# Komputerowe-Projektowanie-Lekow/pmarlo

Hardware: AMD Instinct MI355X
Metric: frames/sec featurize->TICA->k-means->T-matrix, 1Mx64 synth; ITS rel-err (higher is better)
Workload: dtype f64; 1 GPU; synthetic 1000000 frames x 64 f32 features per GPU (AR(1) latents), TICA->10, k=500 (10 Lloyd iterations), lag=10, row-normalised T; frames_per_gpu=1000000, features=64, tica_dim=10, k=500, lag=10, kmeans_iters=10, parallelism=shards1

## Files before the change

include/msmhip.h:

```cpp
#ifndef MSMHIP_H
#define MSMHIP_H

#include <stddef.h>
#include <stdint.h>

#ifdef __cplusplus
extern "C" {
#endif

typedef struct msm_ctx msm_ctx;
typedef struct msm_event msm_event;
typedef struct msm_graph msm_graph;

typedef enum {
    MSM_OK = 0,
    MSM_ERR_INVALID = 1,
    MSM_ERR_HIP = 2,
    MSM_ERR_NOMEM = 3,
    MSM_ERR_UNSUPPORTED = 4,
    MSM_ERR_NOCONV = 5
} msm_status;

typedef enum { MSM_F32 = 0, MSM_F64 = 1 } msm_dtype;

// ... 93 lines not shown
msm_status msm_lagged_moments_onesided(msm_ctx* ctx, const void* d_x, msm_dtype dtype, int64_t n, int F,
                                       int64_t ld, const int64_t* h_seg_start, const int64_t* h_seg_stop,
                                       int n_seg, int lag, const double* d_shift, int assume_finite,
                                       double* d_moments);

msm_status msm_onesided_tica_eigenvalues(msm_ctx* ctx, const double* d_moments, int F, double clip,
                                         double* d_eigvals);

msm_status msm_moments_from_lagged(msm_ctx* ctx, const void* d_x, msm_dtype dtype, int64_t n, int F, int64_t ld,
                                   const int64_t* h_seg_start, const int64_t* h_seg_stop, int n_seg, int lag,
                                   const double* d_shift, const double* d_moments, double* d_sums);

msm_status msm_tica_solve(msm_ctx* ctx, const double* d_moments, const double* d_scale, int F,
                          double epsilon, int kinetic_map, double* d_eigvals, double* d_coeffs,
                          double* d_mean, int* d_rank);

msm_status msm_project(msm_ctx* ctx, const void* d_x, msm_dtype dtype, int64_t n, int F, int64_t ld,
                       const double* d_mu, const double* d_inv_sigma, const double* d_mean2,
                       const double* d_w, int d, int64_t ldw, double* d_y, int64_t ldy, double* d_absmax);

msm_status msm_project_finite(msm_ctx* ctx, const void* d_x, msm_dtype dtype, int64_t n, int F, int64_t ld,
                              const double* d_mu, const double* d_inv_sigma, const double* d_mean2,
                              const double* d_w, int d, int64_t ldw, double* d_y, int64_t ldy, double* d_absmax);

msm_status msm_eigh(msm_ctx* ctx, const double* d_a, int n, double* d_w, double* d_v, int* d_sweeps);


msm_status msm_kmeans_assign(msm_ctx* ctx, const void* d_x, msm_dtype dtype, int64_t n, int d,
                             int64_t ld, const double* d_centers, int k,
                             const double* d_mean, const double* d_std,
// ... 150 lines not shown
```

pmarlo_amd/_lib.py:

```python

from __future__ import annotations

import ctypes as C
from pathlib import Path

__all__ = ["lib", "load", "LIB_PATH", "check", "MsmError", "DECLARED_SYMBOLS"]

LIB_PATH = Path(__file__).resolve().parent / "csrc" / "libmsmhip.so"

MSM_OK, MSM_ERR_INVALID, MSM_ERR_HIP, MSM_ERR_NOMEM, MSM_ERR_UNSUPPORTED, MSM_ERR_NOCONV = range(6)
MSM_F32, MSM_F64 = 0, 1


class MsmError(RuntimeError):
    """A HIP-side failure reported through the C ABI."""


_vp = C.c_void_p
_i32 = C.c_int
_i64 = C.c_int64
_sz = C.c_size_t
_f64 = C.c_double
_pp = C.POINTER(C.c_void_p)

# ... 26 lines not shown
    "msm_featurize_sasa": (_i32, [_vp, _vp, _i64, _i32, _vp, _vp, _i32, _vp]),
    "msm_hbond_presence": (_i32, [_vp, _vp, _i64, _i32, _vp, _i32, C.c_float, C.c_float, _vp]),
    "msm_dssp": (_i32, [_vp, _vp, _i64, _i32, _vp, _vp, _vp, _i32, _vp]),
    "msm_count_transitions": (_i32, [_vp, _vp, _i64, _vp, _vp, _i32, _i32, _i32, _i32, _vp, _vp]),
    "msm_count_transitions_weighted": (
        _i32, [_vp, _vp, _vp, _i64, _vp, _vp, _i32, _i32, _i32, _i32, _vp, _vp]),
    "msm_count_transitions_lagscan": (_i32, [_vp, _vp, _i64, _vp, _vp, _i32, _vp, _i32, _i32, _vp, _vp]),
    "msm_state_counts": (_i32, [_vp, _vp, _i64, _i32, _vp]),
    "msm_column_moments_partial": (_i32, [_vp, _vp, _i32, _i64, _i32, _i64, _vp, _vp, _vp]),
    "msm_moments_finalize": (_i32, [_vp, _vp, _vp, _i32, _i32, _vp, _vp, _vp]),
    "msm_column_moments": (_i32, [_vp, _vp, _i32, _i64, _i32, _i64, _i32, _vp, _vp, _vp]),
    "msm_column_minmax": (_i32, [_vp, _vp, _i32, _i64, _i32, _i64, _vp, _vp, _vp]),
    "msm_standardise_params": (_i32, [_vp, _vp, _vp, _i32, _f64, _i32, _vp, _vp, _vp]),
    "msm_lagged_moments": (_i32, [_vp, _vp, _i32, _i64, _i32, _i64, _vp, _vp, _i32, _i32, _vp, _i32, _vp]),
    "msm_tica_solve": (_i32, [_vp, _vp, _vp, _i32, _f64, _i32, _vp, _vp, _vp, _vp]),
    "msm_lagged_moments_reversible": (_i32, [_vp, _vp, _i32, _i64, _i32, _i64, _vp, _vp, _i32, _i32, _vp, _i32, _vp]),
    "msm_lagged_moments_onesided": (_i32, [_vp, _vp, _i32, _i64, _i32, _i64, _vp, _vp, _i32, _i32, _vp, _i32, _vp]),
    "msm_onesided_tica_eigenvalues": (_i32, [_vp, _vp, _i32, _f64, _vp]),
    "msm_moments_from_lagged": (_i32, [_vp, _vp, _i32, _i64, _i32, _i64, _vp, _vp, _i32, _i32, _vp, _vp, _vp]),
    "msm_project": (_i32, [_vp, _vp, _i32, _i64, _i32, _i64, _vp, _vp, _vp, _vp, _i32, _i64, _vp, _i64, _vp]),
    "msm_project_finite": (_i32, [_vp, _vp, _i32, _i64, _i32, _i64, _vp, _vp, _vp, _vp, _i32, _i64, _vp, _i64, _vp]),
    "msm_eigh": (_i32, [_vp, _vp, _i32, _vp, _vp, _vp]),
    "msm_kmeans_assign": (_i32, [_vp, _vp, _i32, _i64, _i32, _i64, _vp, _i32, _vp, _vp, _vp, _vp]),
    "msm_kmeans_fit": (_i32, [_vp, _vp, _i32, _i64, _i32, _i64, _vp, _vp, _i32, C.c_uint64, _i32, _i32, _f64, _vp, _vp]),
    "msm_kmeans_fit_begin": (
        _i32, [_vp, _vp, _i32, _i64, _i32, _i64, _vp, _vp, _i32, C.c_uint64, _i32, _f64, _f64, _vp, _vp, _i32]),
    "msm_kmeans_accumulate": (_i32, [_vp, _vp, _i32, _i64, _i32, _i64, _vp, _i32, _vp, _vp, _vp, _vp, _vp]),
    "msm_kmeans_update": (_i32, [_vp, _vp, _vp, _i32, _i32, _vp, _vp, _i32]),
    "msm_comm_unique_id": (_i32, [_vp, _sz]),
    "msm_comm_init": (_i32, [_vp, _i32, _i32, _vp, _sz, _pp]),
# ... 104 lines not shown
```

pmarlo_amd/csrc/eig.hip:

```cpp
#include "common.h"

#ifdef MSM_JACOBI_STAMPS
__device__ unsigned long long g_jacobi_stamps[8];
#define JSTAMP(i)                                                                          \
    do {                                                                                   \
        unsigned long long t__;                                                            \
        asm volatile("s_memtime %0\n\ts_waitcnt lgkmcnt(0)" : "=s"(t__)::"memory");       \
        acc__[i] += t__ - last__;                                                          \
        last__ = t__;                                                                      \
    } while (0)
#define JSTAMP_INIT unsigned long long acc__[8] = {0, 0, 0, 0, 0, 0, 0, 0}; unsigned long long last__; asm volatile("s_memtime %0\n\ts_waitcnt lgkmcnt(0)" : "=s"(last__)::"memory");
#define JSTAMP_FLUSH if (threadIdx.x == 0) { for (int i__ = 0; i__ < 8; ++i__) g_jacobi_stamps[i__] += acc__[i__]; }
#else
#define JSTAMP(i)
#define JSTAMP_INIT
#define JSTAMP_FLUSH
#endif

namespace {

constexpr int kEigThreads = 1024;
constexpr int kMaxPairs = 128;

struct JacobiShared {
// ... 528 lines not shown
    const int r1 = 8 * nblocks - 32;
    return __popc(w0 ^ (w0 >> 1)) + __popc(bits ^ ((bits >> 1) | ((w0 & 1u) << (r1 - 1))));
}

__device__ __forceinline__ double bcast_lane(double x, int j) {
    const long long b = __double_as_longlong(x);
    const int lo = __builtin_amdgcn_readlane((int)b, j), hi = __builtin_amdgcn_readlane((int)(b >> 32), j);
    return __longlong_as_double(((long long)hi << 32) | (unsigned)lo);
}
template <typename F>
__device__ __forceinline__ void hh_for_groups(int sub, int k, F&& body) {
#pragma unroll
    for (int g = 0; g < 2; ++g)
        if (sub + 32 * g + 24 > k) body(g);
}
__device__ __forceinline__ void householder_phase(double* A, double* QT, int n, TriShared* ts) {
    static_assert(kEigThreads == 1024, "householder_phase deals the rows of A and Q' over sixteen waves");
    constexpr int ld = kTriLd;
    const int lane = threadIdx.x & 63, wave = __builtin_amdgcn_readfirstlane(threadIdx.x >> 6);
    const bool in = lane < n;
    const bool is_a = wave < 8;
#ifdef MSM_TRI_NOQ
    const bool is_q = false;
#else
    const bool is_q = !is_a;
#endif
    const int sub = wave & 7;
    double* part = ts->part[wave];
    const double* parts = ts->part[is_a ? 0 : 8];
    double2* vw = ts->vw[sub];
    double m[8];
#pragma unroll
    for (int t = 0; t < 8; ++t) {
        const int j = sub + 8 * t;
        m[t] = (in && j < n) ? (is_a ? A[j * ld + lane] : (j == lane ? 1.0 : 0.0)) : 0.0;
    }
    auto q_partial = [&](int c) {
        if (__builtin_amdgcn_readfirstlane(ts->taupub[c & 1] != 0.0)) {
            const double* vp = ts->vpub[c & 1];
            double s0 = 0.0, s1 = 0.0;
// ... 31 lines not shown
        const double* rowc = A + c * ld;
        double xi = rowc[in ? lane : 0];
        const double alpha = rowc[c + 1];
        if (wave == 0 && lane == c) ts->d[c] = xi;
        const bool actc = in && lane > c;
        if (!actc) xi = 0.0;
        const double sigma = wave_sum_all(lane > c + 1 ? xi * xi : 0.0);
        const bool nz = sigma != 0.0;
        const double h2 = fma(alpha, alpha, sigma);
        const double rs = nr_rsqrt(nz ? h2 : 1.0);
        const double beta = nz ? -copysign(h2 * rs, alpha) : alpha;
        tau = nz ? (beta - alpha) * -copysign(rs, alpha) : 0.0;
        const double scal = nr_rcp(nz ? alpha - beta : 1.0);
        vi = actc ? (lane == c + 1 ? 1.0 : (nz ? xi * scal : 0.0)) : 0.0;
        if (wave == 0) {
            ts->vpub[c & 1][lane] = vi;
            if (lane == 0) { ts->e[c] = beta; ts->taupub[c & 1] = tau; }
        }
        vw[lane].x = vi;
    };
    LSTAMP_INIT
    double vi = 0.0, tau = 0.0;
    if (is_a && n > 2) reflector(0, vi, tau);
    for (int k = 0; k + 2 < n; ++k) {
        LSTAMP(16);
        const bool act = in && lane > k;
        if (is_a) {
            double s0 = 0.0, s1 = 0.0;
            hh_for_groups(sub, k, [&](int g) {
                double v[4];
#pragma unroll
                for (int u = 0; u < 4; ++u) v[u] = vw[sub + 32 * g + 8 * u].x;
// ... 119 lines not shown
        for (int t = 0; t < 8; ++t)
            if (lane == sub + 8 * t && lane < n) ts->inv[lane] = nr_rsqrt(m[t]);
    }
    __syncthreads();
    if (what == 1 && in) {
#pragma unroll
        for (int t = 0; t < 8; ++t) {
            const int i = sub + 8 * t;
            if (i < n) W[lane * ld + i] = m[t] * ts->inv[i];
        }
    }
    __syncthreads();
    return true;
}

__device__ __forceinline__ bool tridiag_eigh(double* A, double* Q, double* X, int n, int ld, TriShared* ts, double orth_tol) {
    const int tid = threadIdx.x, nt = blockDim.x, lane = tid & 63, wave = tid >> 6;
    if (n == 1) {
        if (tid == 0) { ts->lam[0] = A[0]; A[0] = 1.0; }
        __syncthreads();
        return true;
    }
    if (ld != kTriLd) return false;
    TSTAMP_INIT
    if (tid == 0) ts->bad = 0;
    __syncthreads();
    TSTAMP(0);
    householder_phase(A, Q, n, ts);
    TSTAMP(1);
    __syncthreads();
    TSTAMP(2);
    {
        const double dl = lane < n ? ts->d[lane] : 0.0, el = lane < n ? ts->e[lane] : 0.0;
        double an = fmax(fabs(dl), fabs(el));
#pragma unroll
        for (int off = 32; off > 0; off >>= 1) an = fmax(an, __shfl_xor(an, off, 64));
        double sc = 1.0;
        if (an > 0.0 && an < 1e300) { int ex; (void)frexp(an, &ex); sc = ldexp(1.0, -ex); }
        const double ds = dl * sc, es = el * sc;
        const double em = lane > 0 && lane < n ? ts->e[lane - 1] * sc : 0.0;
        const double rad = fabs(em) + (lane + 1 < n ? fabs(es) : 0.0);
        double gl = lane < n ? ds - rad : 1e300, gu = lane < n ? ds + rad : -1e300;
#pragma unroll
        for (int off = 32; off > 0; off >>= 1) {
            gl = fmin(gl, __shfl_xor(gl, off, 64));
            gu = fmax(gu, __shfl_xor(gu, off, 64));
        }
        __syncthreads();
        if (wave == 0) {
            if (lane < n) { ts->d[lane] = ds; ts->e[lane] = es; ts->de[lane] = make_double2(ds, em * em); }
            else ts->de[lane] = make_double2(8.0, 0.0);
            if (lane < 8) ts->de[kTriMax + lane] = make_double2(8.0, 0.0);
            if (lane == 0) {
                if (!(an < 1e300)) ts->bad = 1;
                ts->scale = sc;
                const double bn = fmax(fabs(gl), fabs(gu));
                const double pad = 4.0 * n * 2.220446049250313e-16 * bn + 1e-290;
                ts->gl = gl - pad;
                ts->gu = gu + pad;
            }
        }
    }
    __syncthreads();
    TSTAMP(3);
    if (ts->bad) return false;
    if (tid < 8 * kTriMax && wave * 8 < n) {
        const int i = tid >> 3, t = tid & 7;
        const int nblocks = (n + 7) >> 3;
        double lo = ts->gl, hi = ts->gu;
        const double frac = (double)(t + 1) * (1.0 / 9.0);
        for (int it = 0; it < 20; ++it) {
            const double x = fma(hi - lo, frac, lo);
            const int c = sturm_count(ts, nblocks, x);
            double nlo = c <= i ? x : lo, nhi = c > i ? x : hi;
            nlo = hw_max_f64(nlo, mov_dpp64<0xB1>(nlo)); nhi = hw_min_f64(nhi, mov_dpp64<0xB1>(nhi));
            nlo = hw_max_f64(nlo, mov_dpp64<0x4E>(nlo)); nhi = hw_min_f64(nhi, mov_dpp64<0x4E>(nhi));
            nlo = hw_max_f64(nlo, mov_dpp64<0x141>(nlo)); nhi = hw_min_f64(nhi, mov_dpp64<0x141>(nhi));
            lo = nlo;
            hi = nhi;
        }
        if (i < n && t == 0) ts->lam[i] = 0.5 * (lo + hi);
    }
    __syncthreads();
    TSTAMP(4);
    const double tiny = 1e-290;
    double* Xc = X + (lane < n ? lane : 0);
    double* Ac = A + (lane < n ? lane : 0);
    const double lamb = ts->lam[lane < n ? lane : 0];
    if (wave == 0 && lane < n) {
        double q = ts->de[0].x - lamb;
        Xc[0] = q;
        for (int j0 = 1; j0 < n; j0 += 8) {
            double2 r[8];
#pragma unroll
            for (int u = 0; u < 8; ++u) r[u] = ts->de[j0 + u];
#pragma unroll
            for (int u = 0; u < 8; ++u) {
                if (j0 + u < n) {
                    if (fabs(q) < tiny) q = -tiny;
                    q = fma(-r[u].y, nr_rcp(q), r[u].x - lamb);
                    Xc[(j0 + u) * ld] = q;
                }
            }
        }
    } else if (wave == 1 && lane < n) {
        double r = ts->de[n - 1].x - lamb;
        if (fabs(r) < tiny) r = -tiny;
        double ir = nr_rcp(r);
        Ac[(n - 1) * ld] = ir;
        for (int j0 = n - 2; j0 >= 0; j0 -= 8) {
            double dj[8], e2[8];
#pragma unroll
            for (int u = 0; u < 8; ++u) {
                const int j = j0 - u >= 0 ? j0 - u : 0;
                dj[u] = ts->de[j].x;
                e2[u] = ts->de[j + 1].y;
            }
#pragma unroll
            for (int u = 0; u < 8; ++u) {
                if (j0 - u >= 0) {
                    r = fma(-e2[u], ir, dj[u] - lamb);
                    if (fabs(r) < tiny) r = -tiny;
                    ir = nr_rcp(r);
                    Ac[(j0 - u) * ld] = ir;
                }
            }
        }
    }
    __syncthreads();
    int kk = n - 1;
    if (wave < 2 && lane < n) {
        double gbest = fabs(Xc[(n - 1) * ld]);
        for (int j0 = n - 2; j0 >= 0; j0 -= 8) {
            double g[8];
#pragma unroll
            for (int u = 0; u < 8; ++u) {
                const int j = j0 - u >= 0 ? j0 - u : 0;
                g[u] = fabs(fma(-ts->de[j + 1].y, Ac[(j + 1) * ld], Xc[j * ld]));
            }
#pragma unroll
            for (int u = 0; u < 8; ++u)
                if (j0 - u >= 0 && g[u] <= gbest) { gbest = g[u]; kk = j0 - u; }
        }
    }
    __syncthreads();
    if (wave == 0 && lane < n) {
        double z = 1.0, nrm2 = 1.0;
        for (int j0 = n - 2; j0 >= 0; j0 -= 8) {
            double f[8];
#pragma unroll
            for (int u = 0; u < 8; ++u) {
                const int j = j0 - u >= 0 ? j0 - u : 0;
                double qq = Xc[j * ld];
                if (fabs(qq) < tiny) qq = -tiny;
                f[u] = -(ts->e[j] * nr_rcp(qq));
            }
#pragma unroll
            for (int u = 0; u < 8; ++u) {
                if (j0 - u >= 0 && j0 - u < kk) {
                    z = f[u] * z;
                    Xc[(j0 - u) * ld] = z;
                    nrm2 = fma(z, z, nrm2);
                }
            }
        }
        Xc[kk * ld] = 1.0;
        ts->praw[lane] = nrm2;
    } else if (wave == 1 && lane < n) {
        double z = 1.0, nrm2 = 0.0;
        for (int j0 = 0; j0 + 1 < n; j0 += 8) {
            double f[8];
#pragma unroll
            for (int u = 0; u < 8; ++u) {
                const int j = j0 + u + 1 < n ? j0 + u : 0;
                f[u] = -(ts->e[j] * Ac[(j + 1) * ld]);
            }
#pragma unroll
            for (int u = 0; u < 8; ++u) {
                if (j0 + u + 1 < n && j0 + u >= kk) {
                    z = f[u] * z;
                    Xc[(j0 + u + 1) * ld] = z;
                    nrm2 = fma(z, z, nrm2);
                }
            }
        }
        ts->uq[lane] = nrm2;
    }
    __syncthreads();
    if (tid < n) {
        const double nrm2 = ts->praw[tid] + ts->uq[tid];
        const bool ok = nrm2 > 0.0 && nrm2 < 1e300;
        ts->inv[tid] = nr_rsqrt(ok ? nrm2 : 1.0);
        if (!ok) ts->bad = 1;
    }
    __syncthreads();
    TSTAMP(5);
    {
        double worst = 0.0;
        bool bad = false;
        for (int e0 = tid; e0 < n * n; e0 += nt) {
            const int j = e0 / n, i = e0 - j * n;
            const double x0 = X[j * ld + i];
            const double xm = j > 0 ? ts->e[j - 1] * X[(j - 1) * ld + i] : 0.0;
            const double xp = j + 1 < n ? ts->e[j] * X[(j + 1) * ld + i] : 0.0;
            const double tx = fma(ts->d[j] - ts->lam[i], x0, xm + xp) * ts->inv[i];
            bad = bad || !(fabs(tx) <= 1e-10);
        }
        const int jj = lane & 15, g = lane >> 4;
        const int tiles = (n + 15) >> 4;
        for (int t = wave; t < tiles * tiles; t += nt >> 6) {
            const int a0 = (t / tiles) * 16, b0 = (t - (t / tiles) * tiles) * 16;
            if (b0 > a0) continue;
            const bool aok = a0 + jj < n, bok = b0 + jj < n;
            const int ai = aok ? a0 + jj : 0, bi = bok ? b0 + jj : 0;
            const double sa = ts->inv[ai], sb = ts->inv[bi];
            tri_v4f64 acc = {0.0, 0.0, 0.0, 0.0};
            for (int k0 = 0; k0 < n; k0 += 16) {
                double a[4], b[4];
#pragma unroll
                for (int u = 0; u < 4; ++u) {
                    const bool kok = k0 + 4 * u + g < n;
                    const int k = kok ? k0 + 4 * u + g : 0;
                    a[u] = X[k * ld + ai] * sa;
                    b[u] = X[k * ld + bi] * sb;
                    if (!(aok && kok)) a[u] = 0.0;
                    if (!(bok && kok)) b[u] = 0.0;
                }
#pragma unroll
                for (int u = 0; u < 4; ++u) acc = __builtin_amdgcn_mfma_f64_16x16x4f64(a[u], b[u], acc, 0, 0, 0);
            }
#pragma unroll
            for (int r = 0; r < 4; ++r) {
                const int row = a0 + g + 4 * r, col = b0 + jj;
                if (row < n && col < n) worst = fmax(worst, fabs(acc[r] - (row == col ? 1.0 : 0.0)));
            }
        }
        if (bad) worst = 1e300;
#pragma unroll
        for (int off = 32; off > 0; off >>= 1) worst = fmax(worst, __shfl_xor(worst, off, 64));
        if (lane == 0) ts->red[wave] = worst;
        __syncthreads();
        worst = 0.0;
        for (int w = 0; w < nt / 64; ++w) worst = fmax(worst, ts->red[w]);
        TSTAMP(6);
        if (ts->bad || !(worst <= orth_tol)) return false;
    }
    mfma_mm<true, false>(A, Q, X, n, n, n, ld, ts->inv);
    if (tid < n) ts->lam[tid] /= ts->scale;
    __syncthreads();
    TSTAMP(7);
    return true;
}

struct TicaWork {
    double *A, *V, *B1, *B2, *ev, *mean, *isc;
    int* order;
};

template <int lds_mats>
__global__ __launch_bounds__(kEigThreads) void tica_solve_kernel(
    const double* __restrict__ mom, const double* __restrict__ scale, int n, int ld, double epsilon, int kinetic_map,
    TicaWork wk, double* __restrict__ out_eig, double* __restrict__ out_W, double* __restrict__ out_mean,
    int* __restrict__ out_rank) {
    extern __shared__ __attribute__((aligned(16))) unsigned char smem_raw[];
    __shared__ JacobiShared sh;
    __shared__ TriShared ts;
    const int tid = threadIdx.x, nt = blockDim.x;
    double* lds = reinterpret_cast<double*>(smem_raw);
    const size_t mat = (size_t)n * ld;
    double *A, *V, *B1, *B2;
    if constexpr (lds_mats >= 2) { A = lds; V = lds + mat; } else { A = wk.A; V = wk.V; }
    if constexpr (lds_mats >= 4) { B1 = lds + 2 * mat; B2 = lds + 3 * mat; } else { B1 = wk.B1; B2 = wk.B2; }

    const double* M00 = mom;
    const double* M0t = mom + (size_t)n * n;
    const double* sx = M0t + (size_t)n * n;
    const double* sy = sx + n;
// ... 102 lines not shown
        __syncthreads();
    }
    mfma_mm<false, false>(A, B1, B2, n, rank, n, ld);
    mfma_mm<true, false>(V, B2, A, rank, rank, n, ld);
    for (int e = tid; e < rank * rank; e += nt) {
        const int i = e / rank, j = e - i * rank;
        A[i * ld + j] = 0.5 * (V[i * ld + j] + V[j * ld + i]);
    }
    __syncthreads();
    KSTAMP(10);
    const double* Vec = V;
    bool fast = false;
    if (kFused && rank <= kTriMax) {
        for (int e = tid; e < rank * rank; e += nt) wk.A[e] = A[(e / rank) * ld + (e % rank)];
        __syncthreads();
        fast = tridiag_eigh(A, V, B1, rank, ld, &ts, 1e-11);
        if (fast) {
            for (int i = tid; i < rank; i += nt) wk.ev[i] = ts.lam[i];
            Vec = A;
        } else {
            __syncthreads();
            for (int e = tid; e < rank * rank; e += nt) A[(e / rank) * ld + (e % rank)] = wk.A[e];
        }
        __syncthreads();
    }
    if (!fast) {
        jacobi_eigh(A, V, rank, ld, &sh, 40);
        for (int i = tid; i < rank; i += nt) wk.ev[i] = A[i * ld + i];
    }
    __syncthreads();
// ... 18 lines not shown
            const int lane = tid & 63, wave = tid >> 6;
            for (int j = wave; j < rank; j += nt >> 6) {
                double best = lane < n ? fabs(B1[lane * ld + j]) : -1.0;
                int bi = lane;
                double val = lane < n ? B1[lane * ld + j] : 0.0;
#pragma unroll
                for (int off = 1; off < 64; off <<= 1) {
                    const double ob = __shfl_xor(best, off, 64), ov = __shfl_xor(val, off, 64);
                    const int oi = __shfl_xor(bi, off, 64);
                    if (ob > best || (ob == best && oi < bi)) { best = ob; bi = oi; val = ov; }
                }
                if (lane == 0) sgn[j] = val < 0.0 ? -1.0 : 1.0;
            }
        }
        __syncthreads();
        for (int e = tid; e < n * n; e += nt) {
            const int i = e / n, j = e - i * n;
            double v = 0.0;
            if (j < rank) {
                const int c = ord[j];
                v = B1[i * ld + c] * sgn[c];
                if (kinetic_map) v *= evl[c];
            }
            out_W[e] = v;
        }
        for (int j = tid; j < n; j += nt) out_eig[j] = j < rank ? evl[ord[j]] : 0.0;
        KSTAMP(12);
        return;
    }
    sort_desc_abs(wk.ev, rank, wk.order);
    mfma_mm<false, false>(B1, B2, Vec, n, rank, rank, ld);
    canonical_signs(B1, n, rank, ld);
    for (int e = tid; e < n * n; e += nt) {
        const int i = e / n, j = e - i * n;
        double v = 0.0;
        if (j < rank) {
            v = B1[i * ld + wk.order[j]];
            if (kinetic_map) v *= wk.ev[wk.order[j]];
        }
        out_W[e] = v;
    }
    for (int j = tid; j < n; j += nt) out_eig[j] = j < rank ? wk.ev[wk.order[j]] : 0.0;
    KSTAMP(12);
}

template <bool use_lds>
__global__ __launch_bounds__(kEigThreads) void eigh_kernel(const double* __restrict__ Ain, int n, int ld,
                                                          double* gA, double* gV, int* order,
                                                          double* __restrict__ out_w, double* __restrict__ out_v,
                                                          int* __restrict__ out_sweeps) {
    extern __shared__ __attribute__((aligned(16))) unsigned char smem_raw[];
    __shared__ JacobiShared sh;
    const int tid = threadIdx.x, nt = blockDim.x;
    double *A, *V;
    if constexpr (use_lds) { A = reinterpret_cast<double*>(smem_raw); V = A + (size_t)n * ld; }
    else { A = gA; V = gV; }
    for (int e = tid; e < n * n; e += nt) {
// ... 113 lines not shown
            const double b = gw[j];
            rank += (b > a) || (b == a && j < i);
        }
        order[rank] = i;
    }
    __syncthreads();
    for (int j = tid; j < n; j += nt) out_eig[j] = gw[order[j]];
}

size_t jacobi_lds_bytes(int n, int ld) { return (size_t)(n <= kTriMax ? 3 : 2) * n * ld * sizeof(double); }

}

extern "C" {

msm_status msm_tica_solve(msm_ctx* ctx, const double* d_moments, const double* d_scale, int F, double epsilon,
                          int kinetic_map, double* d_eigvals, double* d_coeffs, double* d_mean, int* d_rank) {
    if (!ctx) return MSM_ERR_INVALID;
    MSM_REQUIRE(ctx, F >= 1 && F <= 2 * kMaxPairs, "msm_tica_solve: need 1 <= F <= %d (got %d)", 2 * kMaxPairs, F);
    MSM_REQUIRE(ctx, epsilon >= 0.0, "msm_tica_solve: epsilon must be >= 0");
    MSM_REQUIRE(ctx, d_moments && d_eigvals && d_coeffs && d_mean && d_rank, "msm_tica_solve: NULL pointer");
    const int ld = F <= kTriMax ? kTriLd : (F | 1);
    const size_t mat = (size_t)F * ld;
    const size_t need = (4 * mat + 3 * F) * sizeof(double) + (size_t)F * sizeof(int) + 64;
    msm_status rs = msm_reserve_scratch(ctx, need);
    if (rs != MSM_OK) return rs;
    double* base = (double*)ctx->scratch;
    TicaWork wk;
    wk.A = base; wk.V = base + mat; wk.B1 = base + 2 * mat; wk.B2 = base + 3 * mat;
    wk.ev = base + 4 * mat; wk.mean = wk.ev + F; wk.isc = wk.mean + F; wk.order = (int*)(wk.isc + F);
    const size_t lds_budget = 150 * 1024;
    int lds_mats = 0;
    if (4 * mat * sizeof(double) <= lds_budget) lds_mats = 4;
    else if (2 * mat * sizeof(double) <= lds_budget) lds_mats = 2;
    const size_t lds = (size_t)lds_mats * mat * sizeof(double);
    auto kern = lds_mats == 4 ? tica_solve_kernel<4> : (lds_mats == 2 ? tica_solve_kernel<2> : tica_solve_kernel<0>);
    if (lds > 48 * 1024)
        MSM_HIP(ctx, hipFuncSetAttribute((const void*)kern, hipFuncAttributeMaxDynamicSharedMemorySize, (int)lds));
    hipLaunchKernelGGL(kern, dim3(1), dim3(kEigThreads), lds, ctx->stream, d_moments, d_scale, F, ld, epsilon,
                       kinetic_map, wk, d_eigvals, d_coeffs, d_mean, d_rank);
    MSM_CHECK_LAUNCH(ctx);
    return MSM_OK;
}

msm_status msm_onesided_tica_eigenvalues(msm_ctx* ctx, const double* d_moments, int F, double clip, double* d_eigvals) {
    if (!ctx) return MSM_ERR_INVALID;
    MSM_REQUIRE(ctx, F >= 1 && F <= 2 * kMaxPairs, "msm_onesided_tica_eigenvalues: need 1 <= F <= %d (got %d)",
                2 * kMaxPairs, F);
    MSM_REQUIRE(ctx, d_moments && d_eigvals && clip > 0.0, "msm_onesided_tica_eigenvalues: bad arguments");
    const int ld = F <= kTriMax ? kTriLd : (F | 1);
    const size_t mat = (size_t)F * ld;
    const size_t lds = 4 * mat * sizeof(double);
    const bool use_lds = lds <= 140 * 1024;
    msm_status rs = msm_reserve_scratch(ctx, ((use_lds ? 0 : 4 * mat) + (size_t)F * F + F) * sizeof(double) +
                                                 (size_t)F * sizeof(int) + 64);
    if (rs != MSM_OK) return rs;
    double* gP = (double*)ctx->scratch;
// ... 36 lines not shown
```

pmarlo_amd/device.py:

```python

from __future__ import annotations

import ctypes as C
import os
import sys
from typing import Iterable, Sequence

import numpy as np

from . import _lib
from ._lib import check, lib

__all__ = ["Engine", "DeviceArray", "get_engine", "segments_to_bounds"]


def _dtype_code(dtype: np.dtype) -> int:
    dtype = np.dtype(dtype)
    if dtype == np.float32:
        return _lib.MSM_F32
    if dtype == np.float64:
        return _lib.MSM_F64
    raise TypeError(f"feature matrices must be float32 or float64, got {dtype}")


# ... 425 lines not shown
        return out

    def moments_from_lagged(self, x: DeviceArray, lag: int, shift: DeviceArray, moments: DeviceArray, *, starts=None,
                            stops=None, out: DeviceArray | None = None) -> DeviceArray:
        n, F = x.shape
        if starts is None:
            starts, stops = segments_to_bounds(None, n)
        starts, stops = self._seg_ptrs(starts, stops)
        out = out if out is not None else self.empty((3 * F,), np.float64)
        check(lib.msm_moments_from_lagged(self.handle, x.ptr, _dtype_code(x.dtype), n, F, F, starts.ctypes.data,
                                          stops.ctypes.data, len(starts), int(lag), shift.ptr, moments.ptr, out.ptr),
              self.handle)
        return out

    def tica_solve(self, moments: DeviceArray, F: int, *, scale: DeviceArray | None = None,
                   epsilon: float = 1e-6, kinetic_map: bool = True, out=None):
        if out is not None:
            eig, W, mean, rank = out
        else:
            eig = self.empty((F,), np.float64)
            W = self.empty((F, F), np.float64)
            mean = self.empty((F,), np.float64)
            rank = self.empty((1,), np.int32)
        check(lib.msm_tica_solve(self.handle, moments.ptr, scale.ptr if scale is not None else None, F,
                                 float(epsilon), int(bool(kinetic_map)), eig.ptr, W.ptr, mean.ptr, rank.ptr),
              self.handle)
        return eig, W, mean, rank

    def project(self, x: DeviceArray, mu: DeviceArray, inv_sigma: DeviceArray, W: DeviceArray, d: int, *,
                mean2: DeviceArray | None = None, out: DeviceArray | None = None,
                absmax: DeviceArray | None = None, assume_finite: bool = False) -> DeviceArray:
        n, F = x.shape
        ldw = W.shape[1]
        out = out if out is not None else self.empty((n, d), np.float64)
        fn = lib.msm_project_finite if assume_finite else lib.msm_project
        check(fn(self.handle, x.ptr, _dtype_code(x.dtype), n, F, F, mu.ptr, inv_sigma.ptr,
                 mean2.ptr if mean2 is not None else None, W.ptr, int(d), ldw, out.ptr,
                 out.shape[1], absmax.ptr if absmax is not None else None), self.handle)
        return out

    def eigh(self, a: DeviceArray, want_vectors: bool = True):
# ... 548 lines not shown
```

pmarlo_amd/dist.py:

```python

from __future__ import annotations

import ctypes as C
import os
import time
from dataclasses import dataclass
from pathlib import Path

import numpy as np

from .device import DeviceArray, Engine

__all__ = ["Comm", "NativeComm", "TorchComm", "ShardedMSM", "ShardConfig", "exchange_shapes", "exchange_aliases",
           "torch_exchange_buffers", "bootstrap_id"]


class Comm:

    world = 1
    rank = 0

    def allreduce_sum(self, name: str) -> None: ...
    def allreduce_sum_from(self, name: str, src) -> None: ...
    def allreduce_min(self, name: str) -> None: ...
# ... 272 lines not shown
                raise ValueError("ShardConfig.pairs must list n_features atom pairs")
            self.xyz = x
            self.pairs_d = eng.to_device(np.ascontiguousarray(cfg.pairs, np.int32).reshape(F, 2))
            self.x = eng.empty((n, F), np.float32)
            eng.featurize_distances_into(self.xyz, self.pairs_d, self.x)
        else:
            self.xyz = None
            self.x = x
        if cfg.tica_dim > 0:
            self.mean, self.scale, self.inv_scale = (eng.empty((F,), np.float64) for _ in range(3))
            self.eig = eng.empty((F,), np.float64)
            self.W = eng.empty((F, F), np.float64)
            self.m2 = eng.empty((F,), np.float64)
            self.rank_d = eng.empty((1,), np.int32)
            self.Y = eng.empty((n, d), np.float64)
        else:
            self.Y = self.x
        self.labels = eng.empty((n,), np.int32)
        self.T = eng.empty((k, k), np.float64)
        self.rowsum = eng.empty((k,), np.float64)
        self.diag = eng.empty((1,), np.float64)
        self.km_sums = b["km_acc"].view((k * d,), np.int64)
        self.km_counts = b["km_acc"].view((k,), np.int64, offset_elems=k * d)
        multi_shard = self.comm is not None and (self.comm.world > 1 or self.always_exchange)
        self.km_local = eng.empty((k * d + k,), np.int64) if multi_shard else None
        nbytes = eng.kmeans_image_bytes(n, d)
        self.km_image = eng.empty((nbytes,), np.uint8) if nbytes else None
        self.accum_events: list = []
        self.stage_events: dict = {}
        self.time_accum = False
# ... 19 lines not shown
        multi = comm is not None and (comm.world > 1 or self.always_exchange)
        F, d, k = cfg.n_features, cfg.cluster_dim, cfg.k
        self._stamp("begin")
        if self.xyz is not None:
            eng.featurize_distances_into(self.xyz, self.pairs_d, self.x)
            self._stamp("featurize")
        if cfg.tica_dim > 0:
            eng.lagged_moments(self.x, cfg.lag, b["shift"], assume_finite=True, out=b["lagged"], symmetric=True)
            eng.moments_from_lagged(self.x, cfg.lag, b["shift"], b["lagged"], out=b["mom_sums"])
            if multi:
                comm.allreduce_sum("moments")
            eng.standardise_params(b["mom_sums"], b["shift"], F, float(self.n_total), True,
                                   out=(self.mean, self.scale, self.inv_scale))
            self._stamp("moments")
            eng.tica_solve(b["lagged"], F, scale=self.scale, epsilon=1e-6, kinetic_map=True,
                           out=(self.eig, self.W, self.m2, self.rank_d))
            self._stamp("tica_solve")
            eng.project(self.x, b["shift"], self.inv_scale, self.W, d, mean2=self.m2, out=self.Y,
                        absmax=b["fit_state"].view((1,), offset_elems=2), assume_finite=True)
            self._stamp("project")
        eng.kmeans_fit_begin(self.Y, k, seed=cfg.seed, n_total=self.n_total, tol2=0.0, centers=b["centers"],
                             state=b["fit_state"], absmax_ready=cfg.tica_dim > 0)
        if multi:
            if comm.rank != 0:
                b["centers"].fill_bytes_(0x7F)
            b["start_scale"].copy_from(b["fit_scale"])
            comm.allreduce_min("start")
            b["fit_scale"].copy_from(b["start_scale"])
            comm.reciprocal("fit_inv_scale", "fit_scale")
        acc = self.km_local if self.km_local is not None else b["km_acc"]
        acc.zero_()
# ... 57 lines not shown
```

Baseline: 653.7 million frames/s.

## Add leading-eigenpair TICA solve that computes only the kept components

```diff
diff --git a/include/msmhip.h b/include/msmhip.h
--- a/include/msmhip.h
+++ b/include/msmhip.h
@@ -131,6 +131,10 @@
 msm_status msm_tica_solve(msm_ctx* ctx, const double* d_moments, const double* d_scale, int F,
                           double epsilon, int kinetic_map, double* d_eigvals, double* d_coeffs,
                           double* d_mean, int* d_rank);
+
+msm_status msm_tica_solve_leading(msm_ctx* ctx, const double* d_moments, const double* d_scale, int F,
+                                  double epsilon, int kinetic_map, int n_keep, double* d_eigvals,
+                                  double* d_coeffs, double* d_mean, int* d_rank);
 
 msm_status msm_project(msm_ctx* ctx, const void* d_x, msm_dtype dtype, int64_t n, int F, int64_t ld,
                        const double* d_mu, const double* d_inv_sigma, const double* d_mean2,
diff --git a/pmarlo_amd/_lib.py b/pmarlo_amd/_lib.py
--- a/pmarlo_amd/_lib.py
+++ b/pmarlo_amd/_lib.py
@@ -64,6 +64,7 @@
     "msm_standardise_params": (_i32, [_vp, _vp, _vp, _i32, _f64, _i32, _vp, _vp, _vp]),
     "msm_lagged_moments": (_i32, [_vp, _vp, _i32, _i64, _i32, _i64, _vp, _vp, _i32, _i32, _vp, _i32, _vp]),
     "msm_tica_solve": (_i32, [_vp, _vp, _vp, _i32, _f64, _i32, _vp, _vp, _vp, _vp]),
+    "msm_tica_solve_leading": (_i32, [_vp, _vp, _vp, _i32, _f64, _i32, _i32, _vp, _vp, _vp, _vp]),
     "msm_lagged_moments_reversible": (_i32, [_vp, _vp, _i32, _i64, _i32, _i64, _vp, _vp, _i32, _i32, _vp, _i32, _vp]),
     "msm_lagged_moments_onesided": (_i32, [_vp, _vp, _i32, _i64, _i32, _i64, _vp, _vp, _i32, _i32, _vp, _i32, _vp]),
     "msm_onesided_tica_eigenvalues": (_i32, [_vp, _vp, _i32, _f64, _vp]),
diff --git a/pmarlo_amd/csrc/eig.hip b/pmarlo_amd/csrc/eig.hip
--- a/pmarlo_amd/csrc/eig.hip
+++ b/pmarlo_amd/csrc/eig.hip
@@ -566,6 +566,7 @@
     for (int g = 0; g < 2; ++g)
         if (sub + 32 * g + 24 > k) body(g);
 }
+template <bool kKeepQ = true>
 __device__ __forceinline__ void householder_phase(double* A, double* QT, int n, TriShared* ts) {
     static_assert(kEigThreads == 1024, "householder_phase deals the rows of A and Q' over sixteen waves");
     constexpr int ld = kTriLd;
@@ -575,7 +576,7 @@
 #ifdef MSM_TRI_NOQ
     const bool is_q = false;
 #else
-    const bool is_q = !is_a;
+    const bool is_q = kKeepQ && !is_a;
 #endif
     const int sub = wave & 7;
     double* part = ts->part[wave];
@@ -637,8 +638,13 @@
         const double scal = nr_rcp(nz ? alpha - beta : 1.0);
         vi = actc ? (lane == c + 1 ? 1.0 : (nz ? xi * scal : 0.0)) : 0.0;
         if (wave == 0) {
-            ts->vpub[c & 1][lane] = vi;
-            if (lane == 0) { ts->e[c] = beta; ts->taupub[c & 1] = tau; }
+            if constexpr (kKeepQ) {
+                ts->vpub[c & 1][lane] = vi;
+                if (lane == 0) ts->taupub[c & 1] = tau;
+            } else if (in) {
+                QT[c * ld + lane] = lane == c ? tau : vi;
+            }
+            if (lane == 0) ts->e[c] = beta;
         }
         vw[lane].x = vi;
     };
@@ -788,80 +794,64 @@
     return true;
 }
 
-__device__ __forceinline__ bool tridiag_eigh(double* A, double* Q, double* X, int n, int ld, TriShared* ts, double orth_tol) {
-    const int tid = threadIdx.x, nt = blockDim.x, lane = tid & 63, wave = tid >> 6;
-    if (n == 1) {
-        if (tid == 0) { ts->lam[0] = A[0]; A[0] = 1.0; }
-        __syncthreads();
-        return true;
-    }
-    if (ld != kTriLd) return false;
-    TSTAMP_INIT
-    if (tid == 0) ts->bad = 0;
-    __syncthreads();
-    TSTAMP(0);
-    householder_phase(A, Q, n, ts);
-    TSTAMP(1);
-    __syncthreads();
-    TSTAMP(2);
-    {
-        const double dl = lane < n ? ts->d[lane] : 0.0, el = lane < n ? ts->e[lane] : 0.0;
-        double an = fmax(fabs(dl), fabs(el));
-#pragma unroll
-        for (int off = 32; off > 0; off >>= 1) an = fmax(an, __shfl_xor(an, off, 64));
-        double sc = 1.0;
-        if (an > 0.0 && an < 1e300) { int ex; (void)frexp(an, &ex); sc = ldexp(1.0, -ex); }
-        const double ds = dl * sc, es = el * sc;
-        const double em = lane > 0 && lane < n ? ts->e[lane - 1] * sc : 0.0;
-        const double rad = fabs(em) + (lane + 1 < n ? fabs(es) : 0.0);
-        double gl = lane < n ? ds - rad : 1e300, gu = lane < n ? ds + rad : -1e300;
-#pragma unroll
-        for (int off = 32; off > 0; off >>= 1) {
-            gl = fmin(gl, __shfl_xor(gl, off, 64));
-            gu = fmax(gu, __shfl_xor(gu, off, 64));
-        }
-        __syncthreads();
-        if (wave == 0) {
-            if (lane < n) { ts->d[lane] = ds; ts->e[lane] = es; ts->de[lane] = make_double2(ds, em * em); }
-            else ts->de[lane] = make_double2(8.0, 0.0);
-            if (lane < 8) ts->de[kTriMax + lane] = make_double2(8.0, 0.0);
-            if (lane == 0) {
-                if (!(an < 1e300)) ts->bad = 1;
-                ts->scale = sc;
-                const double bn = fmax(fabs(gl), fabs(gu));
-                const double pad = 4.0 * n * 2.220446049250313e-16 * bn + 1e-290;
-                ts->gl = gl - pad;
-                ts->gu = gu + pad;
-            }
-        }
-    }
-    __syncthreads();
-    TSTAMP(3);
-    if (ts->bad) return false;
-    if (tid < 8 * kTriMax && wave * 8 < n) {
-        const int i = tid >> 3, t = tid & 7;
-        const int nblocks = (n + 7) >> 3;
-        double lo = ts->gl, hi = ts->gu;
-        const double frac = (double)(t + 1) * (1.0 / 9.0);
-        for (int it = 0; it < 20; ++it) {
-            const double x = fma(hi - lo, frac, lo);
-            const int c = sturm_count(ts, nblocks, x);
-            double nlo = c <= i ? x : lo, nhi = c > i ? x : hi;
-            nlo = hw_max_f64(nlo, mov_dpp64<0xB1>(nlo)); nhi = hw_min_f64(nhi, mov_dpp64<0xB1>(nhi));
-            nlo = hw_max_f64(nlo, mov_dpp64<0x4E>(nlo)); nhi = hw_min_f64(nhi, mov_dpp64<0x4E>(nhi));
-            nlo = hw_max_f64(nlo, mov_dpp64<0x141>(nlo)); nhi = hw_min_f64(nhi, mov_dpp64<0x141>(nhi));
-            lo = nlo;
-            hi = nhi;
-        }
-        if (i < n && t == 0) ts->lam[i] = 0.5 * (lo + hi);
-    }
-    __syncthreads();
-    TSTAMP(4);
+__device__ __forceinline__ void tri_scale_bounds(int n, TriShared* ts) {
+    const int lane = threadIdx.x & 63, wave = threadIdx.x >> 6;
+    const double dl = lane < n ? ts->d[lane] : 0.0, el = lane < n ? ts->e[lane] : 0.0;
+    double an = fmax(fabs(dl), fabs(el));
+#pragma unroll
+    for (int off = 32; off > 0; off >>= 1) an = fmax(an, __shfl_xor(an, off, 64));
+    double sc = 1.0;
+    if (an > 0.0 && an < 1e300) { int ex; (void)frexp(an, &ex); sc = ldexp(1.0, -ex); }
+    const double ds = dl * sc, es = el * sc;
+    const double em = lane > 0 && lane < n ? ts->e[lane - 1] * sc : 0.0;
+    const double rad = fabs(em) + (lane + 1 < n ? fabs(es) : 0.0);
+    double gl = lane < n ? ds - rad : 1e300, gu = lane < n ? ds + rad : -1e300;
+#pragma unroll
+    for (int off = 32; off > 0; off >>= 1) {
+        gl = fmin(gl, __shfl_xor(gl, off, 64));
+        gu = fmax(gu, __shfl_xor(gu, off, 64));
+    }
+    __syncthreads();
+    if (wave == 0) {
+        if (lane < n) { ts->d[lane] = ds; ts->e[lane] = es; ts->de[lane] = make_double2(ds, em * em); }
+        else ts->de[lane] = make_double2(8.0, 0.0);
+        if (lane < 8) ts->de[kTriMax + lane] = make_double2(8.0, 0.0);
+        if (lane == 0) {
+            if (!(an < 1e300)) ts->bad = 1;
+            ts->scale = sc;
+            const double bn = fmax(fabs(gl), fabs(gu));
+            const double pad = 4.0 * n * 2.220446049250313e-16 * bn + 1e-290;
+            ts->gl = gl - pad;
+            ts->gu = gu + pad;
+        }
+    }
+}
+
+__device__ __forceinline__ double multisect9(const TriShared* ts, int n, int i, int t) {
+    const int nblocks = (n + 7) >> 3;
+    double lo = ts->gl, hi = ts->gu;
+    const double frac = (double)(t + 1) * (1.0 / 9.0);
+    for (int it = 0; it < 20; ++it) {
+        const double x = fma(hi - lo, frac, lo);
+        const int c = sturm_count(ts, nblocks, x);
+        double nlo = c <= i ? x : lo, nhi = c > i ? x : hi;
+        nlo = hw_max_f64(nlo, mov_dpp64<0xB1>(nlo)); nhi = hw_min_f64(nhi, mov_dpp64<0xB1>(nhi));
+        nlo = hw_max_f64(nlo, mov_dpp64<0x4E>(nlo)); nhi = hw_min_f64(nhi, mov_dpp64<0x4E>(nhi));
+        nlo = hw_max_f64(nlo, mov_dpp64<0x141>(nlo)); nhi = hw_min_f64(nhi, mov_dpp64<0x141>(nhi));
+        lo = nlo;
+        hi = nhi;
+    }
+    return 0.5 * (lo + hi);
+}
+
+__device__ __forceinline__ void twisted_vectors(double* A, double* X, int n, int ncols, TriShared* ts) {
+    constexpr int ld = kTriLd;
+    const int tid = threadIdx.x, lane = tid & 63, wave = tid >> 6;
     const double tiny = 1e-290;
-    double* Xc = X + (lane < n ? lane : 0);
-    double* Ac = A + (lane < n ? lane : 0);
-    const double lamb = ts->lam[lane < n ? lane : 0];
-    if (wave == 0 && lane < n) {
+    double* Xc = X + (lane < ncols ? lane : 0);
+    double* Ac = A + (lane < ncols ? lane : 0);
+    const double lamb = ts->lam[lane < ncols ? lane : 0];
+    if (wave == 0 && lane < ncols) {
         double q = ts->de[0].x - lamb;
         Xc[0] = q;
         for (int j0 = 1; j0 < n; j0 += 8) {
@@ -877,7 +867,7 @@
                 }
             }
         }
-    } else if (wave == 1 && lane < n) {
+    } else if (wave == 1 && lane < ncols) {
         double r = ts->de[n - 1].x - lamb;
         if (fabs(r) < tiny) r = -tiny;
         double ir = nr_rcp(r);
@@ -903,7 +893,7 @@
     }
     __syncthreads();
     int kk = n - 1;
-    if (wave < 2 && lane < n) {
+    if (wave < 2 && lane < ncols) {
         double gbest = fabs(Xc[(n - 1) * ld]);
         for (int j0 = n - 2; j0 >= 0; j0 -= 8) {
             double g[8];
@@ -918,7 +908,7 @@
         }
     }
     __syncthreads();
-    if (wave == 0 && lane < n) {
+    if (wave == 0 && lane < ncols) {
         double z = 1.0, nrm2 = 1.0;
         for (int j0 = n - 2; j0 >= 0; j0 -= 8) {
             double f[8];
@@ -940,7 +930,7 @@
         }
         Xc[kk * ld] = 1.0;
         ts->praw[lane] = nrm2;
-    } else if (wave == 1 && lane < n) {
+    } else if (wave == 1 && lane < ncols) {
         double z = 1.0, nrm2 = 0.0;
         for (int j0 = 0; j0 + 1 < n; j0 += 8) {
             double f[8];
@@ -961,66 +951,192 @@
         ts->uq[lane] = nrm2;
     }
     __syncthreads();
-    if (tid < n) {
+    if (tid < ncols) {
         const double nrm2 = ts->praw[tid] + ts->uq[tid];
         const bool ok = nrm2 > 0.0 && nrm2 < 1e300;
         ts->inv[tid] = nr_rsqrt(ok ? nrm2 : 1.0);
         if (!ok) ts->bad = 1;
     }
     __syncthreads();
+}
+
+__device__ __forceinline__ double vectors_defect(const double* X, int n, int ncols, TriShared* ts) {
+    constexpr int ld = kTriLd;
+    const int tid = threadIdx.x, nt = blockDim.x, lane = tid & 63, wave = tid >> 6;
+    double worst = 0.0;
+    bool bad = false;
+    for (int e0 = tid; e0 < n * ncols; e0 += nt) {
+        const int j = e0 / ncols, i = e0 - j * ncols;
+        const double x0 = X[j * ld + i];
+        const double xm = j > 0 ? ts->e[j - 1] * X[(j - 1) * ld + i] : 0.0;
+        const double xp = j + 1 < n ? ts->e[j] * X[(j + 1) * ld + i] : 0.0;
+        const double tx = fma(ts->d[j] - ts->lam[i], x0, xm + xp) * ts->inv[i];
+        bad = bad || !(fabs(tx) <= 1e-10);
+    }
+    const int jj = lane & 15, g = lane >> 4;
+    const int tiles = (ncols + 15) >> 4;
+    for (int t = wave; t < tiles * tiles; t += nt >> 6) {
+        const int a0 = (t / tiles) * 16, b0 = (t - (t / tiles) * tiles) * 16;
+        if (b0 > a0) continue;
+        const bool aok = a0 + jj < ncols, bok = b0 + jj < ncols;
+        const int ai = aok ? a0 + jj : 0, bi = bok ? b0 + jj : 0;
+        const double sa = ts->inv[ai], sb = ts->inv[bi];
+        tri_v4f64 acc = {0.0, 0.0, 0.0, 0.0};
+        for (int k0 = 0; k0 < n; k0 += 16) {
+            double a[4], b[4];
+#pragma unroll
+            for (int u = 0; u < 4; ++u) {
+                const bool kok = k0 + 4 * u + g < n;
+                const int k = kok ? k0 + 4 * u + g : 0;
+                a[u] = X[k * ld + ai] * sa;
+                b[u] = X[k * ld + bi] * sb;
+                if (!(aok && kok)) a[u] = 0.0;
+                if (!(bok && kok)) b[u] = 0.0;
+            }
+#pragma unroll
+            for (int u = 0; u < 4; ++u) acc = __builtin_amdgcn_mfma_f64_16x16x4f64(a[u], b[u], acc, 0, 0, 0);
+        }
+#pragma unroll
+        for (int r = 0; r < 4; ++r) {
+            const int row = a0 + g + 4 * r, col = b0 + jj;
+            if (row < ncols && col < ncols) worst = fmax(worst, fabs(acc[r] - (row == col ? 1.0 : 0.0)));
+        }
+    }
+    if (bad) worst = 1e300;
+#pragma unroll
+    for (int off = 32; off > 0; off >>= 1) worst = fmax(worst, __shfl_xor(worst, off, 64));
+    if (lane == 0) ts->red[wave] = worst;
+    __syncthreads();
+    worst = 0.0;
+    for (int w = 0; w < nt / 64; ++w) worst = fmax(worst, ts->red[w]);
+    return worst;
+}
+
+__device__ __forceinline__ bool tridiag_eigh(double* A, double* Q, double* X, int n, int ld, TriShared* ts, double orth_tol) {
+    const int tid = threadIdx.x, wave = tid >> 6;
+    if (n == 1) {
+        if (tid == 0) { ts->lam[0] = A[0]; A[0] = 1.0; }
+        __syncthreads();
+        return true;
+    }
+    if (ld != kTriLd) return false;
+    TSTAMP_INIT
+    if (tid == 0) ts->bad = 0;
+    __syncthreads();
+    TSTAMP(0);
+    householder_phase(A, Q, n, ts);
+    TSTAMP(1);
+    __syncthreads();
+    TSTAMP(2);
+    tri_scale_bounds(n, ts);
+    __syncthreads();
+    TSTAMP(3);
+    if (ts->bad) return false;
+    if (tid < 8 * kTriMax && wave * 8 < n) {
+        const int i = tid >> 3, t = tid & 7;
+        const double lam = multisect9(ts, n, i, t);
+        if (i < n && t == 0) ts->lam[i] = lam;
+    }
+    __syncthreads();
+    TSTAMP(4);
+    twisted_vectors(A, X, n, n, ts);
     TSTAMP(5);
     {
-        double worst = 0.0;
-        bool bad = false;
-        for (int e0 = tid; e0 < n * n; e0 += nt) {
-            const int j = e0 / n, i = e0 - j * n;
-            const double x0 = X[j * ld + i];
-            const double xm = j > 0 ? ts->e[j - 1] * X[(j - 1) * ld + i] : 0.0;
-            const double xp = j + 1 < n ? ts->e[j] * X[(j + 1) * ld + i] : 0.0;
-            const double tx = fma(ts->d[j] - ts->lam[i], x0, xm + xp) * ts->inv[i];
-            bad = bad || !(fabs(tx) <= 1e-10);
-        }
-        const int jj = lane & 15, g = lane >> 4;
-        const int tiles = (n + 15) >> 4;
-        for (int t = wave; t < tiles * tiles; t += nt >> 6) {
-            const int a0 = (t / tiles) * 16, b0 = (t - (t / tiles) * tiles) * 16;
-            if (b0 > a0) continue;
-            const bool aok = a0 + jj < n, bok = b0 + jj < n;
-            const int ai = aok ? a0 + jj : 0, bi = bok ? b0 + jj : 0;
-            const double sa = ts->inv[ai], sb = ts->inv[bi];
-            tri_v4f64 acc = {0.0, 0.0, 0.0, 0.0};
-            for (int k0 = 0; k0 < n; k0 += 16) {
-                double a[4], b[4];
-#pragma unroll
-                for (int u = 0; u < 4; ++u) {
-                    const bool kok = k0 + 4 * u + g < n;
-                    const int k = kok ? k0 + 4 * u + g : 0;
-                    a[u] = X[k * ld + ai] * sa;
-                    b[u] = X[k * ld + bi] * sb;
-                    if (!(aok && kok)) a[u] = 0.0;
-                    if (!(bok && kok)) b[u] = 0.0;
-                }
-#pragma unroll
-                for (int u = 0; u < 4; ++u) acc = __builtin_amdgcn_mfma_f64_16x16x4f64(a[u], b[u], acc, 0, 0, 0);
-            }
-#pragma unroll
-            for (int r = 0; r < 4; ++r) {
-                const int row = a0 + g + 4 * r, col = b0 + jj;
-                if (row < n && col < n) worst = fmax(worst, fabs(acc[r] - (row == col ? 1.0 : 0.0)));
-            }
-        }
-        if (bad) worst = 1e300;
-#pragma unroll
-        for (int off = 32; off > 0; off >>= 1) worst = fmax(worst, __shfl_xor(worst, off, 64));
-        if (lane == 0) ts->red[wave] = worst;
-        __syncthreads();
-        worst = 0.0;
-        for (int w = 0; w < nt / 64; ++w) worst = fmax(worst, ts->red[w]);
+        const double worst = vectors_defect(X, n, n, ts);
         TSTAMP(6);
         if (ts->bad || !(worst <= orth_tol)) return false;
     }
     mfma_mm<true, false>(A, Q, X, n, n, n, ld, ts->inv);
     if (tid < n) ts->lam[tid] /= ts->scale;
+    __syncthreads();
+    TSTAMP(7);
+    return true;
+}
+
+__device__ __forceinline__ bool tridiag_leading(double* A, double* R, double* X, int n, int nk, TriShared* ts, int* sel,
+                                                double orth_tol) {
+    constexpr int ld = kTriLd;
+    const int tid = threadIdx.x, lane = tid & 63, wave = tid >> 6;
+    TSTAMP_INIT
+    if (tid == 0) ts->bad = 0;
+    __syncthreads();
+    TSTAMP(0);
+    householder_phase<false>(A, R, n, ts);
+    TSTAMP(1);
+    __syncthreads();
+    TSTAMP(2);
+    tri_scale_bounds(n, ts);
+    __syncthreads();
+    TSTAMP(3);
+    if (ts->bad) return false;
+    const int nb = nk + 1;
+    const int ncand = 2 * nb >= n ? n : 2 * nb;
+    auto cand = [&](int c) { return (ncand == n || c < nb) ? c : n - 2 * nb + c; };
+    if (wave * 64 < 8 * ncand) {
+        const int c = tid >> 3, t = tid & 7;
+        const int i = c < ncand ? cand(c) : 0;
+        const double lam = multisect9(ts, n, i, t);
+        if (c < ncand && t == 0) ts->lam[i] = lam;
+    }
+    __syncthreads();
+    TSTAMP(4);
+    if (tid < ncand) {
+        const int i = cand(tid);
+        const double li = ts->lam[i], a = fabs(li);
+        int r = 0;
+        for (int c = 0; c < ncand; ++c) {
+            const int j = cand(c);
+            const double b = fabs(ts->lam[j]);
+            r += (b > a) || (b == a && j < i);
+        }
+        if (r < nk) {
+            sel[r] = i;
+            const double gap = 1e-6 * fmax(fabs(ts->gl), fabs(ts->gu));
+            bool ok = ncand == n || (i != nk && i != n - 1 - nk);
+            if (ok && i > 0) ok = fabs(li - ts->lam[i - 1]) > gap;
+            if (ok && i + 1 < n) ok = fabs(ts->lam[i + 1] - li) > gap;
+            if (!ok) ts->bad = 1;
+        }
+    }
+    __syncthreads();
+    if (ts->bad) return false;
+    {
+        const double ls = tid < nk ? ts->lam[sel[tid]] : 0.0;
+        __syncthreads();
+        if (tid < nk) ts->lam[tid] = ls;
+        __syncthreads();
+    }
+    twisted_vectors(A, X, n, nk, ts);
+    TSTAMP(5);
+    {
+        const double worst = vectors_defect(X, n, nk, ts);
+        TSTAMP(6);
+        if (ts->bad || !(worst <= orth_tol)) return false;
+    }
+    if (wave < nk) {
+        const int ncol = (nk - wave + 15) >> 4;
+        const int row = lane < n ? lane : 0;
+        double x[4];
+#pragma unroll
+        for (int u = 0; u < 4; ++u) {
+            const int c = u < ncol ? wave + 16 * u : wave;
+            x[u] = lane < n ? X[row * ld + c] * ts->inv[c] : 0.0;
+        }
+        for (int k = n - 3; k >= 0; --k) {
+            const double* vk = R + k * ld;
+            const double tau = vk[k];
+            const double v = (lane > k && lane < n) ? vk[row] : 0.0;
+#pragma unroll
+            for (int u = 0; u < 4; ++u)
+                if (u < ncol) x[u] = fma(-tau * wave_sum_all(v * x[u]), v, x[u]);
+        }
+        if (lane < n) {
+#pragma unroll
+            for (int u = 0; u < 4; ++u)
+                if (u < ncol) A[lane * ld + wave + 16 * u] = x[u];
+        }
+    }
+    if (tid < nk) ts->lam[tid] /= ts->scale;
     __syncthreads();
     TSTAMP(7);
     return true;
@@ -1034,7 +1150,7 @@
 template <int lds_mats>
 __global__ __launch_bounds__(kEigThreads) void tica_solve_kernel(
     const double* __restrict__ mom, const double* __restrict__ scale, int n, int ld, double epsilon, int kinetic_map,
-    TicaWork wk, double* __restrict__ out_eig, double* __restrict__ out_W, double* __restrict__ out_mean,
+    int n_keep, TicaWork wk, double* __restrict__ out_eig, double* __restrict__ out_W, double* __restrict__ out_mean,
     int* __restrict__ out_rank) {
     extern __shared__ __attribute__((aligned(16))) unsigned char smem_raw[];
     __shared__ JacobiShared sh;
@@ -1167,6 +1283,44 @@
     if (kFused && rank <= kTriMax) {
         for (int e = tid; e < rank * rank; e += nt) wk.A[e] = A[(e / rank) * ld + (e % rank)];
         __syncthreads();
+        if (full_rank && n_keep < rank) {
+            if (tridiag_leading(A, V, B1, rank, n_keep, &ts, sh.q, 1e-11)) {
+                KSTAMP(11);
+                mfma_mm<false, false>(B1, B2, A, n, n_keep, n, ld);
+                double* sgn = ts.uq;
+                {
+                    const int lane = tid & 63, wave = tid >> 6;
+                    for (int j = wave; j < n_keep; j += nt >> 6) {
+                        double best = lane < n ? fabs(B1[lane * ld + j]) : -1.0;
+                        int bi = lane;
+                        double val = lane < n ? B1[lane * ld + j] : 0.0;
+#pragma unroll
+                        for (int off = 1; off < 64; off <<= 1) {
+                            const double ob = __shfl_xor(best, off, 64), ov = __shfl_xor(val, off, 64);
+                            const int oi = __shfl_xor(bi, off, 64);
+                            if (ob > best || (ob == best && oi < bi)) { best = ob; bi = oi; val = ov; }
+                        }
+                        if (lane == 0) sgn[j] = val < 0.0 ? -1.0 : 1.0;
+                    }
+                }
+                __syncthreads();
+                for (int e = tid; e < n * n; e += nt) {
+                    const int i = e / n, j = e - i * n;
+                    double v = 0.0;
+                    if (j < n_keep) {
+                        v = B1[i * ld + j] * sgn[j];
+                        if (kinetic_map) v *= ts.lam[j];
+                    }
+                    out_W[e] = v;
+                }
+                for (int j = tid; j < n; j += nt) out_eig[j] = j < n_keep ? ts.lam[j] : 0.0;
+                KSTAMP(12);
+                return;
+            }
+            __syncthreads();
+            for (int e = tid; e < rank * rank; e += nt) A[(e / rank) * ld + (e % rank)] = wk.A[e];
+            __syncthreads();
+        }
         fast = tridiag_eigh(A, V, B1, rank, ld, &ts, 1e-11);
         if (fast) {
             for (int i = tid; i < rank; i += nt) wk.ev[i] = ts.lam[i];
@@ -1215,33 +1369,35 @@
             }
         }
         __syncthreads();
+        const int nout = min(rank, n_keep);
         for (int e = tid; e < n * n; e += nt) {
             const int i = e / n, j = e - i * n;
             double v = 0.0;
-            if (j < rank) {
+            if (j < nout) {
                 const int c = ord[j];
                 v = B1[i * ld + c] * sgn[c];
                 if (kinetic_map) v *= evl[c];
             }
             out_W[e] = v;
         }
-        for (int j = tid; j < n; j += nt) out_eig[j] = j < rank ? evl[ord[j]] : 0.0;
+        for (int j = tid; j < n; j += nt) out_eig[j] = j < nout ? evl[ord[j]] : 0.0;
         KSTAMP(12);
         return;
     }
     sort_desc_abs(wk.ev, rank, wk.order);
     mfma_mm<false, false>(B1, B2, Vec, n, rank, rank, ld);
     canonical_signs(B1, n, rank, ld);
+    const int nout = min(rank, n_keep);
     for (int e = tid; e < n * n; e += nt) {
         const int i = e / n, j = e - i * n;
         double v = 0.0;
-        if (j < rank) {
+        if (j < nout) {
             v = B1[i * ld + wk.order[j]];
             if (kinetic_map) v *= wk.ev[wk.order[j]];
         }
         out_W[e] = v;
     }
-    for (int j = tid; j < n; j += nt) out_eig[j] = j < rank ? wk.ev[wk.order[j]] : 0.0;
+    for (int j = tid; j < n; j += nt) out_eig[j] = j < nout ? wk.ev[wk.order[j]] : 0.0;
     KSTAMP(12);
 }
 
@@ -1385,9 +1541,9 @@
 
 extern "C" {
 
-msm_status msm_tica_solve(msm_ctx* ctx, const double* d_moments, const double* d_scale, int F, double epsilon,
-                          int kinetic_map, double* d_eigvals, double* d_coeffs, double* d_mean, int* d_rank) {
-    if (!ctx) return MSM_ERR_INVALID;
+static msm_status tica_solve_launch(msm_ctx* ctx, const double* d_moments, const double* d_scale, int F, double epsilon,
+                                    int kinetic_map, int n_keep, double* d_eigvals, double* d_coeffs, double* d_mean,
+                                    int* d_rank) {
     MSM_REQUIRE(ctx, F >= 1 && F <= 2 * kMaxPairs, "msm_tica_solve: need 1 <= F <= %d (got %d)", 2 * kMaxPairs, F);
     MSM_REQUIRE(ctx, epsilon >= 0.0, "msm_tica_solve: epsilon must be >= 0");
     MSM_REQUIRE(ctx, d_moments && d_eigvals && d_coeffs && d_mean && d_rank, "msm_tica_solve: NULL pointer");
@@ -1409,9 +1565,25 @@
     if (lds > 48 * 1024)
         MSM_HIP(ctx, hipFuncSetAttribute((const void*)kern, hipFuncAttributeMaxDynamicSharedMemorySize, (int)lds));
     hipLaunchKernelGGL(kern, dim3(1), dim3(kEigThreads), lds, ctx->stream, d_moments, d_scale, F, ld, epsilon,
-                       kinetic_map, wk, d_eigvals, d_coeffs, d_mean, d_rank);
+                       kinetic_map, n_keep, wk, d_eigvals, d_coeffs, d_mean, d_rank);
     MSM_CHECK_LAUNCH(ctx);
     return MSM_OK;
+}
+
+msm_status msm_tica_solve(msm_ctx* ctx, const double* d_moments, const double* d_scale, int F, double epsilon,
+                          int kinetic_map, double* d_eigvals, double* d_coeffs, double* d_mean, int* d_rank) {
+    if (!ctx) return MSM_ERR_INVALID;
+    return tica_solve_launch(ctx, d_moments, d_scale, F, epsilon, kinetic_map, F, d_eigvals, d_coeffs, d_mean, d_rank);
+}
+
+msm_status msm_tica_solve_leading(msm_ctx* ctx, const double* d_moments, const double* d_scale, int F, double epsilon,
+                                  int kinetic_map, int n_keep, double* d_eigvals, double* d_coeffs, double* d_mean,
+                                  int* d_rank) {
+    if (!ctx) return MSM_ERR_INVALID;
+    MSM_REQUIRE(ctx, n_keep >= 1 && n_keep <= F, "msm_tica_solve_leading: need 1 <= n_keep <= F (got %d, F = %d)", n_keep,
+                F);
+    return tica_solve_launch(ctx, d_moments, d_scale, F, epsilon, kinetic_map, n_keep, d_eigvals, d_coeffs, d_mean,
+                             d_rank);
 }
 
 msm_status msm_onesided_tica_eigenvalues(msm_ctx* ctx, const double* d_moments, int F, double clip, double* d_eigvals) {
diff --git a/pmarlo_amd/device.py b/pmarlo_amd/device.py
--- a/pmarlo_amd/device.py
+++ b/pmarlo_amd/device.py
@@ -463,7 +463,7 @@
         return out
 
     def tica_solve(self, moments: DeviceArray, F: int, *, scale: DeviceArray | None = None,
-                   epsilon: float = 1e-6, kinetic_map: bool = True, out=None):
+                   epsilon: float = 1e-6, kinetic_map: bool = True, out=None, n_keep: int | None = None):
         if out is not None:
             eig, W, mean, rank = out
         else:
@@ -471,9 +471,14 @@
             W = self.empty((F, F), np.float64)
             mean = self.empty((F,), np.float64)
             rank = self.empty((1,), np.int32)
-        check(lib.msm_tica_solve(self.handle, moments.ptr, scale.ptr if scale is not None else None, F,
-                                 float(epsilon), int(bool(kinetic_map)), eig.ptr, W.ptr, mean.ptr, rank.ptr),
-              self.handle)
+        sp = scale.ptr if scale is not None else None
+        if n_keep is None:
+            st = lib.msm_tica_solve(self.handle, moments.ptr, sp, F, float(epsilon), int(bool(kinetic_map)), eig.ptr,
+                                    W.ptr, mean.ptr, rank.ptr)
+        else:
+            st = lib.msm_tica_solve_leading(self.handle, moments.ptr, sp, F, float(epsilon), int(bool(kinetic_map)),
+                                            int(n_keep), eig.ptr, W.ptr, mean.ptr, rank.ptr)
+        check(st, self.handle)
         return eig, W, mean, rank
 
     def project(self, x: DeviceArray, mu: DeviceArray, inv_sigma: DeviceArray, W: DeviceArray, d: int, *,
diff --git a/pmarlo_amd/dist.py b/pmarlo_amd/dist.py
--- a/pmarlo_amd/dist.py
+++ b/pmarlo_amd/dist.py
@@ -2,6 +2,7 @@
 from __future__ import annotations
 
 import ctypes as C
+import inspect
 import os
 import time
 from dataclasses import dataclass
@@ -310,6 +311,8 @@
             self.m2 = eng.empty((F,), np.float64)
             self.rank_d = eng.empty((1,), np.int32)
             self.Y = eng.empty((n, d), np.float64)
+            self._tica_keep = ({"n_keep": cfg.tica_dim}
+                               if "n_keep" in inspect.signature(eng.tica_solve).parameters else {})
         else:
             self.Y = self.x
         self.labels = eng.empty((n,), np.int32)
@@ -359,7 +362,7 @@
                                    out=(self.mean, self.scale, self.inv_scale))
             self._stamp("moments")
             eng.tica_solve(b["lagged"], F, scale=self.scale, epsilon=1e-6, kinetic_map=True,
-                           out=(self.eig, self.W, self.m2, self.rank_d))
+                           out=(self.eig, self.W, self.m2, self.rank_d), **self._tica_keep)
             self._stamp("tica_solve")
             eng.project(self.x, b["shift"], self.inv_scale, self.W, d, mean2=self.m2, out=self.Y,
                         absmax=b["fit_state"].view((1,), offset_elems=2), assume_finite=True)
```

New measurement: 658.5 million frames/s, median of 6. No clear change (+0.7%).
